# X-rayLaser/DistributedLLM

Measured on NVIDIA H100. Metric: decode tokens/sec LLaMA-7B Q4_0 seq512 bs1, higher is better.
Workload: dtype q4_0*q8_0->f32

## Files before the change

distributedllm_b200/csrc/common.cuh:

```cuda
#pragma once
#include <cuda_runtime.h>
#include <cuda_fp16.h>
#include <cstdint>
#include <cstdio>
#include <cstdarg>
#include <string>

#include "../../include/b200_slice.h"

namespace b200 {

inline std::string & last_error_ref() { static thread_local std::string e; return e; }
inline int fail(int code, const char * fmt, ...) {
    char buf[1024];
    va_list ap; va_start(ap, fmt); vsnprintf(buf, sizeof buf, fmt, ap); va_end(ap);
    last_error_ref() = buf;
    return code;
}
#define B200_CUDA(expr) do { cudaError_t e_ = (expr); if (e_ != cudaSuccess) \
    return b200::fail(B200_ECUDA, "%s failed: %s (%s:%d)", #expr, cudaGetErrorString(e_), __FILE__, __LINE__); } while (0)

__device__ __forceinline__ float fmul(float a, float b) { return __fmul_rn(a, b); }
__device__ __forceinline__ float fadd(float a, float b) { return __fadd_rn(a, b); }
__device__ __forceinline__ float fsub(float a, float b) { return __fsub_rn(a, b); }
__device__ __forceinline__ float ffma(float a, float b, float c) { return __fmaf_rn(a, b, c); }
__device__ __forceinline__ float h2f(uint16_t h) { return __half2float(__ushort_as_half(h)); }
__device__ __forceinline__ uint16_t f2h(float f) { return __half_as_ushort(__float2half_rn(f)); }

__device__ __forceinline__ uint32_t smem_u32(const void * p) { return (uint32_t) __cvta_generic_to_shared(p); }

__device__ __forceinline__ void mbar_init(uint64_t * bar, uint32_t count) {
    asm volatile("mbarrier.init.shared::cta.b64 [%0], %1;" :: "r"(smem_u32(bar)), "r"(count) : "memory");
}
__device__ __forceinline__ void mbar_fence_init() {
    asm volatile("fence.mbarrier_init.release.cluster;" ::: "memory");
}
__device__ __forceinline__ void mbar_arrive(uint64_t * bar) {
    asm volatile("{ .reg .b64 st; mbarrier.arrive.shared::cta.b64 st, [%0]; }" :: "r"(smem_u32(bar)) : "memory");
}
__device__ __forceinline__ void mbar_arrive_expect_tx(uint64_t * bar, uint32_t bytes) {
    asm volatile("{ .reg .b64 st; mbarrier.arrive.expect_tx.shared::cta.b64 st, [%0], %1; }"
                 :: "r"(smem_u32(bar)), "r"(bytes) : "memory");
}
__device__ __forceinline__ bool mbar_try_wait(uint64_t * bar, uint32_t parity) {
    uint32_t ok;
    asm volatile("{ .reg .pred p; mbarrier.try_wait.parity.shared::cta.b64 p, [%1], %2; selp.u32 %0, 1, 0, p; }"
                 : "=r"(ok) : "r"(smem_u32(bar)), "r"(parity) : "memory");
    return ok != 0;
}
__device__ __forceinline__ void mbar_wait(uint64_t * bar, uint32_t parity) {
    while (!mbar_try_wait(bar, parity)) { }
}
__device__ __forceinline__ void bulk_g2s(void * dst_smem, const void * src_gmem, uint32_t bytes, uint64_t * bar) {
    uint64_t pol;
    asm volatile("createpolicy.fractional.L2::evict_first.b64 %0, 1.0;" : "=l"(pol));
    asm volatile("cp.async.bulk.shared::cluster.global.mbarrier::complete_tx::bytes.L2::cache_hint [%0], [%1], %2, [%3], %4;"
                 :: "r"(smem_u32(dst_smem)), "l"(src_gmem), "r"(bytes), "r"(smem_u32(bar)), "l"(pol) : "memory");
}
__device__ __forceinline__ float4 ldg_keep(const float * p) {
    uint64_t pol; float4 v;
    asm volatile("createpolicy.fractional.L2::evict_last.b64 %0, 1.0;" : "=l"(pol));
    asm volatile("ld.global.L2::cache_hint.v4.f32 {%0, %1, %2, %3}, [%4], %5;"
                 : "=f"(v.x), "=f"(v.y), "=f"(v.z), "=f"(v.w) : "l"(p), "l"(pol));
    return v;
}
__device__ __forceinline__ void grid_dep_wait()   { asm volatile("griddepcontrol.wait;" ::: "memory"); }
__device__ __forceinline__ void grid_dep_launch() { asm volatile("griddepcontrol.launch_dependents;" ::: "memory"); }

__device__ __forceinline__ unsigned long long gtime() { unsigned long long t; asm volatile("mov.u64 %0, %%globaltimer;" : "=l"(t)); return t; }
#define B200_TRACE(ptr, slot) do { if (ptr) (ptr)[((size_t) blockIdx.y * gridDim.x + blockIdx.x) * 8 + (slot)] = b200::gtime(); } while (0)

__device__ __forceinline__ void named_bar_sync(int id, int nthreads) {
    asm volatile("bar.sync %0, %1;" :: "r"(id), "r"(nthreads) : "memory");
}

}
```

distributedllm_b200/csrc/kernels.cuh:

```cuda
#pragma once
#include "common.cuh"

namespace b200 {

constexpr int kWT_F16 = 1, kWT_Q4_0 = 2, kWT_Q4_1 = 3, kWT_Q5_0 = 6, kWT_Q5_1 = 7, kWT_Q8_0 = 8;
constexpr int kQ4Chunk = 576, kQ41Chunk = 640, kQ50Chunk = 704, kQ51Chunk = 768, kQ8Chunk = 1088;
constexpr int kWPC = 4;
constexpr int kConsumers = kWPC * 32;
constexpr int kQS = 4;
constexpr float kMagic = 12582912.0f;
constexpr int kMagicI = 0x4B400000;

struct WtTraits {
    int block_bytes;
    int chunk_bytes;
    bool is_signed;
    bool min_plane;
    bool high_plane;
    bool q8_1;
    float act_scale;
};
__host__ __device__ constexpr WtTraits wt_traits(int wt) {
    return wt == kWT_Q4_0 ? WtTraits{18, kQ4Chunk, true, false, false, false, 0.0625f}
         : wt == kWT_Q4_1 ? WtTraits{20, kQ41Chunk, false, true, false, true, 0.0625f}
         : wt == kWT_Q5_0 ? WtTraits{22, kQ50Chunk, true, false, true, false, 0.125f}
         : wt == kWT_Q5_1 ? WtTraits{24, kQ51Chunk, false, true, true, true, 0.125f}
         : wt == kWT_Q8_0 ? WtTraits{34, kQ8Chunk, true, false, false, false, 1.0f}
         :                  WtTraits{0, 0, false, false, false, false, 0.0f};
}
__host__ __device__ constexpr bool wt_block_quant(int wt) { return wt_traits(wt).block_bytes != 0; }
__host__ __device__ constexpr int chunk_bytes(int wt) { return wt_traits(wt).chunk_bytes; }
__host__ __device__ constexpr bool wt_nibbles(int wt) { return wt == kWT_Q4_0 || wt == kWT_Q4_1 || wt == kWT_Q5_0 || wt == kWT_Q5_1; }
__host__ __device__ constexpr bool wt_q8_1(int wt) { return wt_traits(wt).q8_1; }
__host__ __device__ constexpr float wt_act_scale(int wt) { return wt_traits(wt).act_scale; }
__host__ __device__ constexpr int wt_scale_off(int wt) { return wt == kWT_Q8_0 ? 1024 : (wt_traits(wt).high_plane ? 640 : 512); }
__host__ __device__ constexpr int wt_min_off(int wt) { return wt_scale_off(wt) + 64; }
static_assert(chunk_bytes(kWT_Q4_0) == 32 * 18 && chunk_bytes(kWT_Q4_1) == 32 * 20 && chunk_bytes(kWT_Q5_0) == 32 * 22 &&
              chunk_bytes(kWT_Q5_1) == 32 * 24 && chunk_bytes(kWT_Q8_0) == 32 * 34, "a chunk holds the file's bytes, nothing added");
static_assert(kQ50Chunk % 16 == 0 && kQ51Chunk % 16 == 0, "a ring stage stays one bulk copy");

__device__ __forceinline__ uint32_t spread4_hi(uint32_t b) { return (b * 0x10204080u) & 0x80808080u; }

struct PackedW {
    const uint8_t * data;
    int wtype, rows, K, nb, nbq, TR, n_tiles;
    long long tile_bytes;
};

struct RepackArgs {
    const uint8_t * src[3];
    int mode, wtype, rows_per_src, nb, nbq, TR, n_tiles;
    uint8_t * dst;
};

__global__ void k_repack(RepackArgs a) {
    const int cb = chunk_bytes(a.wtype), words = cb / 4;
    const long long total = (long long) a.n_tiles * a.nbq * a.TR * words;
    for (long long i = blockIdx.x * (long long) blockDim.x + threadIdx.x; i < total; i += (long long) gridDim.x * blockDim.x) {
        const int wi = (int)(i % words);
        long long c = i / words;
        const int rg = (int)(c % a.TR); c /= a.TR;
        const int q = (int)(c % a.nbq);
        const int tile = (int)(c / a.nbq);
        const int gi = tile * a.TR + rg;
        int s, sg;
        if (a.mode == 1)      { const int gps = a.rows_per_src / 8; s = gi / gps; sg = gi % gps; }
        else if (a.mode == 2) { s = gi & 1; sg = gi >> 1; }
        else                  { s = 0; sg = gi; }
        const int bsz = wt_traits(a.wtype).block_bytes;
        uint32_t out = 0;
        const bool src_ok = s < 3 && a.src[s] != nullptr;
        if (wt_traits(a.wtype).high_plane) {
            const bool q51 = a.wtype == kWT_Q5_1;
            const int qh_off = q51 ? 4 : 2, qs_off = qh_off + 4;
            if (wi < 128) {
                const int lane = wi >> 2, bq = wi & 3, r = lane >> 2, w = lane & 3;
                const int row = sg * 8 + r, b = q * 4 + bq;
                if (src_ok && row < a.rows_per_src && b < a.nb) {
                    const uint16_t * p = (const uint16_t *)(a.src[s] + ((long long) row * a.nb + b) * bsz + qs_off + 4 * w);
                    out = (uint32_t) p[0] | ((uint32_t) p[1] << 16);
                }
            } else if (wi < 160) {
                const int lane = wi - 128, r = lane >> 2, w = lane & 3, row = sg * 8 + r;
                for (int bq = 0; bq < 4; bq++) {
                    const int b = q * 4 + bq;
                    if (src_ok && row < a.rows_per_src && b < a.nb) {
                        const uint16_t * p = (const uint16_t *)(a.src[s] + ((long long) row * a.nb + b) * bsz + qh_off);
                        const uint32_t qh = (uint32_t) p[0] | ((uint32_t) p[1] << 16);
                        out |= (((qh >> (4 * w)) & 15u) | (((qh >> (16 + 4 * w)) & 15u) << 4)) << (8 * bq);
                    }
                }
            } else {
                const int sel = (wi - 160) >> 4;
                const int h0 = ((wi - 160) & 15) * 2;
                uint32_t v[2] = {0, 0};
                for (int k = 0; k < 2; k++) {
                    const int r = (h0 + k) >> 2, bq = (h0 + k) & 3, row = sg * 8 + r, b = q * 4 + bq;
                    if (src_ok && row < a.rows_per_src && b < a.nb)
                        v[k] = *(const uint16_t *)(a.src[s] + ((long long) row * a.nb + b) * bsz + 2 * sel);
                }
// ... 1013 lines not shown
    for (int i = 0; i < nwarp; i++) S += redd[i];
    const float inv = (float)(1.0 / S);
    for (int t = tid; t < tcount; t += blockDim.x) p16[t] = f2h(fmul(sc[t], inv));
    __syncthreads();

    const int npT = T & ~31;
    const int g = tid / D, c = tid - g * D;
    if (g < 4) {
        float acc[8] = {0.f, 0.f, 0.f, 0.f, 0.f, 0.f, 0.f, 0.f};
        const uint16_t * v = vcb + h * D + c;
        const int lim = min(npT, tcount);
        for (int base = 8 * g; base < lim; base += 32) {
            #pragma unroll
            for (int l = 0; l < 8; l++) {
                const int t = base + l;
                if (t < lim) acc[l] = ffma(h2f(v[(size_t) t * E]), h2f(p16[t]), acc[l]);
            }
        }
        #pragma unroll
        for (int l = 0; l < 8; l++) part[(g * D + c) * 8 + l] = acc[l];
    }
    __syncthreads();
    if (tid < D) {
        float vv[8];
        #pragma unroll
        for (int l = 0; l < 8; l++) {
            const float a0 = fadd(part[(0 * D + tid) * 8 + l], part[(2 * D + tid) * 8 + l]);
            const float a1 = fadd(part[(1 * D + tid) * 8 + l], part[(3 * D + tid) * 8 + l]);
            vv[l] = fadd(a0, a1);
        }
        const float t0 = fadd(vv[0], vv[4]), t1 = fadd(vv[1], vv[5]), t2 = fadd(vv[2], vv[6]), t3 = fadd(vv[3], vv[7]);
        double sumf = (double) fadd(fadd(t0, t1), fadd(t2, t3));
        const uint16_t * v = vcb + h * D + tid;
        for (int t = npT; t < tcount; t++) sumf += (double) fmul(h2f(v[(size_t) t * E]), h2f(p16[t]));
        a.out[(size_t) n * E + h * D + tid] = (float) sumf;
    }
}

struct Attn128Args {
    const float * qkv;
    const uint16_t * q16;
    uint16_t * kc; uint16_t * vc;
    const int * n_past; int E, H, N, n0;
    const float2 * cs; const uint16_t * texp;
    float * out;
    int * aq_out; float * da_out; int out_nbq; float out_dscale;
    int out_soff;
    int n_ctx; float kq_scale;
    unsigned long long * trace;
    const int2 * cols; size_t sess_stride;
    const int * col_T;
    int pf_rows;
    int lut_smem;
};

constexpr int kAttnRow = 272;

__device__ __forceinline__ void cp_async16(void * dst_smem, const void * src) {
    asm volatile("cp.async.cg.shared.global [%0], [%1], 16;" :: "r"(smem_u32(dst_smem)), "l"(src) : "memory");
}
__device__ __forceinline__ void cp_async_wait_all() {
    asm volatile("cp.async.commit_group;" ::: "memory");
    asm volatile("cp.async.wait_group 0;" ::: "memory");
}

__device__ __forceinline__ void cluster_sync_all() {
    asm volatile("barrier.cluster.arrive.release.aligned;" ::: "memory");
    asm volatile("barrier.cluster.wait.acquire.aligned;" ::: "memory");
}
__device__ __forceinline__ void cluster_arrive_relaxed() { asm volatile("barrier.cluster.arrive.relaxed.aligned;" ::: "memory"); }
__device__ __forceinline__ void cluster_wait()           { asm volatile("barrier.cluster.wait.acquire.aligned;" ::: "memory"); }
__device__ __forceinline__ uint32_t dsmem_addr(const void * local, int rank) {
    uint32_t r;
    asm volatile("mapa.shared::cluster.u32 %0, %1, %2;" : "=r"(r) : "r"(smem_u32(local)), "r"(rank));
    return r;
}
__device__ __forceinline__ void dsmem_st(uint32_t addr, float v) {
    asm volatile("st.shared::cluster.f32 [%0], %1;" :: "r"(addr), "f"(v) : "memory");
}
__device__ __forceinline__ void dsmem_st4(uint32_t addr, float4 v) {
    asm volatile("st.shared::cluster.v4.f32 [%0], {%1, %2, %3, %4};" :: "r"(addr), "f"(v.x), "f"(v.y), "f"(v.z), "f"(v.w) : "memory");
}

template <bool FUSE>
__global__ void __cluster_dims__(4, 1, 1) __launch_bounds__(256) k_attn128(const Attn128Args a) {
    extern __shared__ __align__(16) uint8_t smem[];
    __shared__ __align__(16) uint16_t q16s[128], k16s[128], v16s[128];
    __shared__ double redd[8]; __shared__ float redf[8];
    __shared__ __align__(16) float partl[4 * 8 * 32];
    __shared__ __align__(8) uint64_t lutbar;
    if (threadIdx.x == 0) { B200_TRACE(a.trace, 0); grid_dep_launch(); }
    cluster_arrive_relaxed();
    if (!FUSE) grid_dep_wait();
    const int h = blockIdx.x >> 2, g = blockIdx.x & 3, ny = blockIdx.y, n = a.n0 + ny, E = a.E;
    int T, tcount, pos;
    uint16_t * kc = a.kc, * vc = a.vc;
    if (a.cols) {
        const int2 c = a.cols[n]; pos = c.y; tcount = pos + 1; T = (!FUSE && a.col_T) ? a.col_T[n] : tcount;
        kc += (size_t) c.x * a.sess_stride; vc += (size_t) c.x * a.sess_stride;
    }
    else { const int n_past = *a.n_past; T = n_past + a.N; tcount = n_past + n + 1; pos = n_past + n; }
    float * sc = (float *) smem;
    uint16_t * p16 = (uint16_t *)(sc + ((T + 3) & ~3));
    const int tid = threadIdx.x, warp = tid >> 5, lane = tid & 31;
    uint8_t * Ks = smem + ((((size_t)((a.n_ctx + 3) & ~3) * 4 + (size_t)((a.n_ctx + 7) & ~7) * 2) + 15) & ~(size_t) 15);
    uint8_t * Vs = Ks + (size_t) a.pf_rows * kAttnRow;
// ... 144 lines not shown
        for (int tb = 8 * g + l; tb < lim; tb += 128) {
            uint4 vv4[4];
            #pragma unroll
            for (int u = 0; u < 4; u++) {
                const int t = tb + 32 * u;
                const int i = ((t >> 5) << 3) + l;
                const uint16_t * vrow = (FUSE && t == pos) ? v16s : (i < npf ? (const uint16_t *)(Vs + (size_t) i * kAttnRow)
                                                                              : vc + (size_t) t * E + h * 128);
                vv4[u] = t < lim ? *(const uint4 *)(vrow + 8 * cg) : make_uint4(0, 0, 0, 0);
            }
            #pragma unroll
            for (int u = 0; u < 4; u++) {
                const int t = tb + 32 * u;
                if (t < lim) {
                    const uint32_t u4[4] = {vv4[u].x, vv4[u].y, vv4[u].z, vv4[u].w};
                    const float p = h2f(p16[t]);
                    #pragma unroll
                    for (int e = 0; e < 8; e++) {
                        const uint16_t vh = (uint16_t)(u4[e >> 1] >> (16 * (e & 1)));
                        acc[e] = ffma(h2f(vh), p, acc[e]);
                    }
                }
            }
        }
        const uint32_t dst = dsmem_addr(partl + (g * 8 + l) * 32 + 8 * (cg & 3), cg >> 2);
        dsmem_st4(dst, make_float4(acc[0], acc[1], acc[2], acc[3]));
        dsmem_st4(dst + 16, make_float4(acc[4], acc[5], acc[6], acc[7]));
    }
    __syncthreads();
    cluster_sync_all();
    if (threadIdx.x == 0) B200_TRACE(a.trace, 7);

    if (tid < 32) {
        const int c = 32 * g + tid;
        float vv[8];
        #pragma unroll
        for (int l = 0; l < 8; l++) {
            const float p0 = partl[(0 * 8 + l) * 32 + tid], p1 = partl[(1 * 8 + l) * 32 + tid];
            const float p2 = partl[(2 * 8 + l) * 32 + tid], p3 = partl[(3 * 8 + l) * 32 + tid];
            vv[l] = fadd(fadd(p0, p2), fadd(p1, p3));
        }
        const float t0 = fadd(vv[0], vv[4]), t1 = fadd(vv[1], vv[5]), t2 = fadd(vv[2], vv[6]), t3 = fadd(vv[3], vv[7]);
        double sumf = (double) fadd(fadd(t0, t1), fadd(t2, t3));
        for (int t = npT; t < tcount; t++) {
            const uint16_t vh = (FUSE && t == pos) ? v16s[c] : (FUSE ? ((const uint16_t *)(Vt + (size_t)(t - npT) * 64))[tid]
                                                                     : vc[(size_t) t * E + h * 128 + c]);
            sumf += (double) fmul(h2f(vh), h2f(p16[t]));
        }
        const float ov = (float) sumf;
        a.out[(size_t) n * E + h * 128 + c] = ov;
        if (a.aq_out) warp_quant_block(ov, lane, a.aq_out + (size_t) n * a.out_nbq * 32, a.da_out + (size_t) n * a.out_nbq * 4,
                                       4 * h + g, a.out_dscale, a.out_soff);
    }
    if (threadIdx.x == 0) B200_TRACE(a.trace, 3);
}

struct PeerRecvArgs {
    MailboxHdr * mine;
    const uint2 * inbox;
    size_t slot_elems;
    int * peer_ack;
    float * dst; int count;
};

__global__ void __launch_bounds__(1024) k_peer_recv(const PeerRecvArgs a) {
    if (threadIdx.x == 0) grid_dep_launch();
    grid_dep_wait();
    const int s = a.mine->seq_in + 1;
    const uint2 * src = a.inbox + (size_t)(s & (kMbSlots - 1)) * a.slot_elems;
    const unsigned long long t0 = gtime();
    for (int i = blockIdx.x * blockDim.x + threadIdx.x; i < a.count; i += gridDim.x * blockDim.x) {
        uint2 v = ld_ll(src + i);
        while ((int) v.y != s) {
            if (gtime() - t0 > kMbTimeoutNs) { a.mine->err = 1; break; }
            v = ld_ll(src + i);
        }
        a.dst[i] = __uint_as_float(v.x);
    }
    __syncthreads();
    if (threadIdx.x == 0) {
        if (gridDim.x == 1 || atomicAdd(&a.mine->cnt_recv, 1) == (int) gridDim.x - 1) {
            a.mine->cnt_recv = 0;
            a.mine->seq_in = s;
            st_relaxed_sys(a.peer_ack, s);
        }
    }
}

struct PeerSendArgs {
    MailboxHdr * mine;
    uint2 * peer_inbox;
    size_t slot_elems;
    const float * src; int count;
};

__global__ void __launch_bounds__(1024) k_peer_send(const PeerSendArgs a) {
    if (threadIdx.x == 0) grid_dep_launch();
    grid_dep_wait();
    const int s = a.mine->seq_out + 1;
    if (threadIdx.x == 0) mb_wait_slot_free(a.mine, s);
    __syncthreads();
    uint2 * dst = a.peer_inbox + (size_t)(s & (kMbSlots - 1)) * a.slot_elems;
    for (int i = blockIdx.x * blockDim.x + threadIdx.x; i < a.count; i += gridDim.x * blockDim.x) st_ll(dst + i, a.src[i], s);
    __syncthreads();
    if (threadIdx.x == 0) {
        if (gridDim.x == 1 || atomicAdd(&a.mine->cnt_send, 1) == (int) gridDim.x - 1) { a.mine->cnt_send = 0; a.mine->seq_out = s; }
// ... 189 lines not shown
```

distributedllm_b200/csrc/runtime.cu:

```cuda
#include "kernels.cuh"
#include "kquant.cuh"
#include "fastgemm2.cuh"
#include "ggjt_file.hpp"

#include <algorithm>
#include <atomic>
#include <chrono>
#include <climits>
#include <cmath>
#include <condition_variable>
#include <dlfcn.h>
#include <cstdlib>
#include <map>
#include <memory>
#include <mutex>
#include <thread>
#include <type_traits>
#include <vector>

namespace b200 {

constexpr int kSmemLimit = 226 * 1024;

struct LayerW {
    PackedW qkv{}, wo{}, w13{}, w2{};
    PackedW qkv_more[2]{}; int qkv_row[2] = {0, 0};
    uint16_t * f_q = nullptr, * f_k = nullptr, * f_v = nullptr, * f_o = nullptr, * f_1 = nullptr, * f_2 = nullptr, * f_3 = nullptr;
    float * attn_norm = nullptr, * ffn_norm = nullptr;
};

struct GraphKey { const float * in; float * out; int host; bool operator<(const GraphKey & o) const {
    return in != o.in ? in < o.in : (out != o.out ? out < o.out : host < o.host); } };

}

using namespace b200;

struct b200_slice {
    int device = 0, n_sm = 132;
    cudaStream_t stream = nullptr;
    int E = 0, H = 0, D = 0, FF = 0, L = 0, first_layer = 0, n_ctx = 512, wtype = 0;
    int n_sessions = 1, cur = 0;
    std::vector<int> past;
    int * d_npast = nullptr;
    size_t sess_stride = 0;
    struct Seg { int session, past, count, col; };
    std::vector<Seg> segs; std::vector<int> h_pass;
    int * d_pass = nullptr; const int2 * cols = nullptr; const int * col_T = nullptr; const int2 * d_segs = nullptr;
    const AttnTile * d_tiles = nullptr; int n_tiles = 0, tile_rows = 0;
    std::vector<LayerW> layers;
    std::vector<void *> allocs;
    uint16_t * kc = nullptr, * vc = nullptr, * q16 = nullptr;
    float * xa = nullptr, * xb = nullptr, * qkv = nullptr, * att = nullptr, * ffin = nullptr, * gate = nullptr;
    float * d_in = nullptr, * d_out = nullptr, * h_in = nullptr, * h_out = nullptr;
    float2 * cs = nullptr; uint16_t * texp = nullptr, * tsilu = nullptr;
    int * aq_att = nullptr, * aq_gate = nullptr; float * da_att = nullptr, * da_gate = nullptr;
    int nbqE = 0, nbqF = 0;
    int soffE = 0, soffF = 0;
    int * aq_x = nullptr; float * da_x = nullptr; int * nq_counter = nullptr; double * nq_partial = nullptr;
    std::map<GraphKey, cudaGraphExec_t> graphs;
    cudaEvent_t ev0 = nullptr, ev1 = nullptr; bool timed = false;
    int64_t launches = 0, weight_bytes = 0;
    bool use_ring = true, use_graph = true, use_pdl = false, use_nq = true, f16_ring = true, use_tiled_attn = true, f16_mc = true; int f16_mc_cols = 4;
    bool skip_attention = false;
    bool attn_lut_smem = true;
    bool fast_prefill = false; int fast_min_tokens = 32; uint16_t * xh = nullptr;
    int opt_ns = 0, opt_cta_per_sm = 0, opt_nc = 0, opt_pre = 3, opt_nomath = 0;
    float ema_token_ms = 0.f;
    std::mutex mu;
    bool profiling = false; int cur_class = 0;
    std::vector<cudaEvent_t> prof_ev; std::vector<int> prof_cls; size_t prof_used = 0;
    cudaEvent_t mark[2] = {nullptr, nullptr};
    unsigned long long * trace = nullptr; int trace_next = 0; std::vector<int> trace_cls, trace_ctas;
    void * nccl_comm = nullptr; int pp_rank = 0, pp_world = 1; float * d_final = nullptr;
    uint8_t * mb_block = nullptr; size_t mb_slot_floats = 0;
    uint8_t * mb_next = nullptr, * mb_prev = nullptr; bool mb_on = false;
    bool send_pending = false; PeerSendArgs send_args{}; int send_ctas = 1;
    bool fold_send = false, use_fold = true;
    int * kq_aq = nullptr; float * kq_ad = nullptr;
    std::map<GraphKey, cudaGraphExec_t> pp_graphs;
    const b200_stream * owner = nullptr;
};

namespace b200 {

static int env_int(const char * name, int dflt) { const char * v = getenv(name); return v ? atoi(v) : dflt; }

template <typename T> static int dev_alloc(b200_slice * s, T ** p, size_t n) {
    void * q = nullptr;
    cudaError_t e = cudaMalloc(&q, n * sizeof(T));
    if (e != cudaSuccess) return fail(B200_ECUDA, "cudaMalloc(%zu) failed: %s", n * sizeof(T), cudaGetErrorString(e));
    s->allocs.push_back(q); *p = (T *) q; return 0;
}

static void prof_begin(b200_slice * s) {
    if (!s->profiling) return;
    if (s->prof_used + 2 > s->prof_ev.size()) {
        for (int i = 0; i < 2; i++) { cudaEvent_t e; cudaEventCreate(&e); s->prof_ev.push_back(e); }
    }
    cudaEventRecord(s->prof_ev[s->prof_used], s->stream);
}
static void prof_end(b200_slice * s) {
    if (!s->profiling) return;
    cudaEventRecord(s->prof_ev[s->prof_used + 1], s->stream);
    s->prof_cls.push_back(s->cur_class);
    s->prof_used += 2;
}

template <typename K, typename... A>
static int launch(b200_slice * s, K kern, dim3 grid, dim3 block, size_t smem, const A &... args) {
    cudaLaunchConfig_t cfg{};
    cfg.gridDim = grid; cfg.blockDim = block; cfg.dynamicSmemBytes = smem; cfg.stream = s->stream;
    cudaLaunchAttribute at[1];
    at[0].id = cudaLaunchAttributeProgrammaticStreamSerialization;
    at[0].val.programmaticStreamSerializationAllowed = 1;
    cfg.attrs = at; cfg.numAttrs = s->use_pdl ? 1 : 0;
    prof_begin(s);
    B200_CUDA(cudaLaunchKernelEx(&cfg, kern, args...));
// ... 195 lines not shown
        void * p = nullptr;
        cudaDriverEntryPointQueryResult qres;
        if (cudaGetDriverEntryPoint("cuTensorMapEncodeTiled", &p, cudaEnableDefault, &qres) == cudaSuccess && qres == cudaDriverEntryPointSuccess)
            fn = (TensorMapEncodeFn) p;
    });
    return fn;
}

template <int WT, int EPI, int NT>
static int launch_fast_gemm_t(b200_slice * s, const PackedW & W, const float * resid, int ldr, float * y, int ldy, int N, int out_rows) {
    TensorMapEncodeFn enc = tensor_map_encode();
    if (!enc) return fail(B200_ECUDA, "cuTensorMapEncodeTiled is not available from this driver");
    CUtensorMap map;
    const cuuint64_t dims[2] = {(cuuint64_t) W.K, (cuuint64_t) N};
    const cuuint64_t strides[1] = {(cuuint64_t) W.K * 2};
    const cuuint32_t box[2] = {64, (cuuint32_t) NT};
    const cuuint32_t estr[2] = {1, 1};
    CUresult cr = enc(&map, CU_TENSOR_MAP_DATA_TYPE_FLOAT16, 2, (void *) s->xh, dims, strides, box, estr, CU_TENSOR_MAP_INTERLEAVE_NONE,
                      CU_TENSOR_MAP_SWIZZLE_128B, CU_TENSOR_MAP_L2_PROMOTION_L2_256B, CU_TENSOR_MAP_FLOAT_OOB_FILL_NONE);
    if (cr != CUDA_SUCCESS) return fail(B200_ECUDA, "cuTensorMapEncodeTiled failed (%d) for K=%d N=%d", (int) cr, W.K, N);
    if (int rc = smem_attr<k_gemm_tc2<WT, EPI, NT>>(s, f2_smem(WT, NT))) return rc;
    FastGemm2Args a{}; a.W = W; a.resid = resid; a.ldr = ldr; a.y = y; a.ldy = ldy; a.N = N; a.out_rows = out_rows; a.tsilu = s->tsilu;
    const int groups = W.n_tiles * W.TR;
    return launch(s, k_gemm_tc2<WT, EPI, NT>, dim3((groups + 15) / 16, (N + NT - 1) / NT, 1), dim3(kF2Threads, 1, 1), f2_smem(WT, NT), a, map);
}

template <int EPI>
static int launch_fast_gemm(b200_slice * s, const PackedW & W, const float * resid, int ldr, float * y, int ldy, int N, int out_rows) {
    const int mtiles = (W.n_tiles * W.TR + 15) / 16;
    const bool wide = (long long) mtiles * ((N + 255) / 256) >= s->n_sm || N <= 128;
    if (W.wtype == kWT_Q4_0) return wide ? launch_fast_gemm_t<kWT_Q4_0, EPI, 256>(s, W, resid, ldr, y, ldy, N, out_rows)
                                         : launch_fast_gemm_t<kWT_Q4_0, EPI, 128>(s, W, resid, ldr, y, ldy, N, out_rows);
    return wide ? launch_fast_gemm_t<kWT_Q8_0, EPI, 256>(s, W, resid, ldr, y, ldy, N, out_rows)
                : launch_fast_gemm_t<kWT_Q8_0, EPI, 128>(s, W, resid, ldr, y, ldy, N, out_rows);
}

struct AttnSmem { int pf_rows; size_t plain, staged, lut, generic; };

static AttnSmem attn_smem(int n_ctx, int D) {
    AttnSmem m;
    const size_t sc = (size_t)((n_ctx + 3) & ~3) * 4 + (size_t)((n_ctx + 7) & ~7) * 2, sc16 = (sc + 15) & ~(size_t) 15;
    m.pf_rows = std::min(8 * ((n_ctx + 31) / 32), 128);
    m.plain = sc16 + 64;
    m.staged = sc16 + (size_t) 2 * m.pf_rows * kAttnRow + 32 * 64 + 64;
    m.lut = m.staged + 65536;
    m.generic = sc + (size_t) 4 * D * 8 * 4 + 64;
    return m;
}

static bool seg_tiled(const b200_slice * s, const b200_slice::Seg & g) {
    return s->D == 128 && s->use_tiled_attn && g.count > 1 && g.past + g.count <= kAttnTMax;
}

static int attention(b200_slice * s, int il, int N, bool preq) {
    if (s->skip_attention) return 0;
    const int E = s->E, H = s->H, D = s->D;
    const size_t sess_off = s->cols ? 0 : (size_t) s->cur * s->sess_stride;
    uint16_t * kc = s->kc + sess_off + (size_t) il * s->n_ctx * E, * vc = s->vc + sess_off + (size_t) il * s->n_ctx * E;
    int * d_npast = s->d_npast + s->cur;
    const AttnSmem am = attn_smem(s->n_ctx, D);
    const float kq_scale = 1.0f / sqrtf((float) E / (float) H);
    int rc;
    if (D != 128) {
        s->cur_class = 1;
        RopeArgs ra{s->qkv, E, H, D, N, d_npast, s->cs, s->q16, kc, vc, s->cols, s->sess_stride};
        if ((rc = launch(s, k_rope_append, dim3((E / 2 + 255) / 256, N, 1), dim3(256, 1, 1), 0, ra))) return rc;
        s->cur_class = 2;
        AttnArgs aa{s->q16, kc, vc, d_npast, E, H, D, N, s->texp, s->att, kq_scale, s->cols, s->sess_stride, s->col_T};
        return launch(s, k_attention, dim3(H, N, 1), dim3(512, 1, 1), am.generic, aa);
    }
    constexpr int kChunk = 1024;
    Attn128Args aa{};
    aa.pf_rows = am.pf_rows;
    aa.qkv = s->qkv; aa.q16 = s->q16; aa.kc = kc; aa.vc = vc; aa.n_past = d_npast; aa.E = E; aa.H = H; aa.N = N;
    aa.cols = s->cols; aa.sess_stride = s->sess_stride;
    aa.cs = s->cs; aa.texp = s->texp; aa.out = s->att;
    aa.n_ctx = s->n_ctx; aa.kq_scale = kq_scale;
    const float dsc = preq ? wt_act_scale(s->wtype) : 0.f;
    if (preq) { aa.aq_out = s->aq_att; aa.da_out = s->da_att; aa.out_nbq = s->nbqE; aa.out_dscale = dsc; aa.out_soff = s->soffE; }
    auto launch_tiled = [&](int t_rows, int n_blocks, const AttnTile * tiles) {
        AttnTiledArgs ta{};
        ta.q16 = s->q16; ta.kc = kc; ta.vc = vc; ta.n_past = d_npast; ta.E = E; ta.H = H; ta.N = N; ta.texp = s->texp; ta.out = s->att;
        if (preq) { ta.aq_out = s->aq_att; ta.da_out = s->da_att; ta.out_nbq = s->nbqE; ta.out_dscale = dsc; ta.out_soff = s->soffE; }
        ta.kq_scale = kq_scale; ta.t_rows = t_rows; ta.t_pad = (t_rows + 31) & ~31;
        ta.tiles = tiles; ta.sess_stride = s->sess_stride;
        const size_t tsm = (size_t) ta.t_rows * kAttnRow + (size_t) kAttnQB * ta.t_pad * 6 + 4 * 8 * 128 * 4 + kAttnQB * 256 + 64;
        if (int e = smem_attr<k_attn128_tiled>(s, kSmemLimit)) return e;
        return launch(s, k_attn128_tiled, dim3(H, n_blocks, 1), dim3(512, 1, 1), tsm, ta);
    };
    auto launch_fused_cols = [&](int c0, int cnt) {
        for (int n0 = 0; n0 < cnt; n0 += kChunk) {
            aa.n0 = c0 + n0;
            if (int e = launch(s, k_attn128<true>, dim3(4 * H, std::min(cnt - n0, kChunk), 1), dim3(256, 1, 1), am.staged, aa)) return e;
        }
        return 0;
    };
    if (s->cols && !s->col_T) {
        s->cur_class = 2;
        return launch_fused_cols(0, N);
    }
    if (s->cols) {
        const std::vector<b200_slice::Seg> & sg = s->segs;
        s->cur_class = 2;
        for (size_t k = 0; k < sg.size();) {
            size_t e = k;
            while (e < sg.size() && sg[e].count == 1) e++;
            if (e > k && (rc = launch_fused_cols(sg[k].col, sg[e - 1].col + 1 - sg[k].col))) return rc;
            k = e + 1;
        }
        s->cur_class = 1;
        for (const b200_slice::Seg & g : sg) {
            if (g.count == 1) continue;
            RopeArgs ra{s->qkv + (size_t) g.col * 3 * E, E, H, D, g.count, d_npast, s->cs, s->q16 + (size_t) g.col * E, kc, vc,
                        s->cols + g.col, s->sess_stride};
            if ((rc = launch(s, k_rope_append, dim3((E / 2 + 255) / 256, g.count, 1), dim3(256, 1, 1), 0, ra))) return rc;
        }
        s->cur_class = 2;
        if (s->n_tiles && (rc = launch_tiled(s->tile_rows, s->n_tiles, s->d_tiles))) return rc;
        aa.col_T = s->col_T;
        for (const b200_slice::Seg & g : sg) {
            if (g.count == 1 || seg_tiled(s, g)) continue;
            for (int n0 = 0; n0 < g.count; n0 += kChunk) {
                aa.n0 = g.col + n0;
                if ((rc = launch(s, k_attn128<false>, dim3(4 * H, std::min(g.count - n0, kChunk), 1), dim3(256, 1, 1), am.plain, aa))) return rc;
            }
        }
        return 0;
    }
    if (N == 1) {
        s->cur_class = 2;
        aa.n0 = 0;
        if (s->trace && s->trace_next < 512) { aa.trace = s->trace + (size_t) s->trace_next * 1024 * 8; s->trace_next++; s->trace_cls.push_back(2); s->trace_ctas.push_back(4 * H); }
        aa.lut_smem = s->attn_lut_smem;
        return launch(s, k_attn128<true>, dim3(4 * H, 1, 1), dim3(256, 1, 1), aa.lut_smem ? am.lut : am.staged, aa);
    }
    s->cur_class = 1;
    RopeArgs ra{s->qkv, E, H, D, N, d_npast, s->cs, s->q16, kc, vc, nullptr, 0};
    if ((rc = launch(s, k_rope_append, dim3((E / 2 + 255) / 256, N, 1), dim3(256, 1, 1), 0, ra))) return rc;
    s->cur_class = 2;
    if (s->use_tiled_attn && s->past[s->cur] + N <= kAttnTMax)
        return launch_tiled(s->past[s->cur] + N, (N + kAttnQB - 1) / kAttnQB, nullptr);
    for (int n0 = 0; n0 < N; n0 += kChunk) {
        aa.n0 = n0;
        const int cnt = N - n0 < kChunk ? N - n0 : kChunk;
        if ((rc = launch(s, k_attn128<false>, dim3(4 * H, cnt, 1), dim3(256, 1, 1), am.plain, aa))) return rc;
    }
    return 0;
}


static int layer_f16(b200_slice * s, int il, int N, const float * cur, float * nxt) {
    const int E = s->E, FF = s->FF;
    const LayerW & Lw = s->layers[il];
    int rc;
    GemvF16Args q{}; q.K = E; q.x = cur; q.ldx = E; q.norm_w = Lw.attn_norm; q.N = N; q.tsilu = s->tsilu;
    q.rows = 3 * E; q.ldy = 3 * E;
    q.W = Lw.f_q; q.y = s->qkv;
    if ((rc = launch_f16<PRO_NORM, EPI_STORE>(s, q))) return rc;
    if ((rc = attention(s, il, N, false))) return rc;
    s->cur_class = 3;
    GemvF16Args o{}; o.K = E; o.x = s->att; o.ldx = E; o.N = N; o.tsilu = s->tsilu;
    o.rows = E; o.W = Lw.f_o; o.resid = cur; o.ldr = E; o.y = s->ffin; o.ldy = E;
    if ((rc = launch_f16<PRO_PLAIN, EPI_RESID>(s, o))) return rc;
    s->cur_class = 4;
    GemvF16Args g{}; g.K = E; g.x = s->ffin; g.ldx = E; g.norm_w = Lw.ffn_norm; g.N = N; g.tsilu = s->tsilu;
    g.rows = FF; g.W = Lw.f_1; g.W2 = Lw.f_3; g.y = s->gate; g.ldy = FF;
    if ((rc = launch_f16<PRO_NORM, EPI_GATE>(s, g))) return rc;
    s->cur_class = 5;
    GemvF16Args w{}; w.K = FF; w.x = s->gate; w.ldx = FF; w.N = N; w.tsilu = s->tsilu;
    w.rows = E; w.W = Lw.f_2; w.resid = s->ffin; w.ldr = E; w.y = nxt; w.ldy = E;
    return launch_f16<PRO_PLAIN, EPI_RESID>(s, w);
}

static int layer_exact(b200_slice * s, int il, int N, const float * cur, float * nxt) {
    const int E = s->E, FF = s->FF;
    const LayerW & Lw = s->layers[il];
    const bool nq = s->use_nq && N == 1 && !s->cols && Lw.wo.n_tiles <= 256 && Lw.wo.n_tiles <= s->n_sm * 2;
    const float dsc = wt_act_scale(s->wtype);
    int rc;
    GemvArgs q{}; q.W = Lw.qkv; q.x = cur; q.ldx = E; q.norm_w = Lw.attn_norm; q.y = s->qkv; q.ldy = 3 * E;
    q.N = N; q.out_rows = 3 * E; q.tsilu = s->tsilu; q.aq_in = s->aq_x; q.da_in = s->da_x; q.in_soff = s->soffE;
    if (N > 1 && (rc = launch_norm_quant(s, cur, E, Lw.attn_norm, N))) return rc;
    if ((rc = N > 1 || (il > 0 && nq) ? launch_gemv<1, PRO_PREQ, EPI_STORE>(s, q) : launch_gemv<1, PRO_NORM, EPI_STORE>(s, q))) return rc;
    if ((rc = attention(s, il, N, true))) return rc;
    s->cur_class = 3;
    GemvArgs o{}; o.W = Lw.wo; o.x = s->att; o.ldx = E; o.resid = cur; o.ldr = E; o.y = s->ffin; o.ldy = E;
    o.N = N; o.out_rows = E; o.tsilu = s->tsilu; o.aq_in = s->aq_att; o.da_in = s->da_att; o.in_soff = s->soffE; o.out_soff = s->soffE;
    o.nq_norm_w = Lw.ffn_norm; o.nq_counter = s->nq_counter; o.nq_partial = s->nq_partial; o.aq_out = s->aq_x; o.da_out = s->da_x; o.out_nbq = s->nbqE; o.out_dscale = dsc;
    if (s->D == 128) rc = nq ? launch_gemv<1, PRO_PREQ, EPI_RESID_NQ>(s, o) : launch_gemv<1, PRO_PREQ, EPI_RESID>(s, o);
    else             rc = nq ? launch_gemv<1, PRO_PLAIN, EPI_RESID_NQ>(s, o) : launch_gemv<1, PRO_PLAIN, EPI_RESID>(s, o);
    if (rc) return rc;
    s->cur_class = 4;
    GemvArgs g{}; g.W = Lw.w13; g.x = s->ffin; g.ldx = E; g.norm_w = Lw.ffn_norm; g.y = s->gate; g.ldy = FF;
    g.N = N; g.out_rows = FF; g.tsilu = s->tsilu; g.aq_in = s->aq_x; g.da_in = s->da_x; g.in_soff = s->soffE; g.out_soff = s->soffF;
    g.aq_out = s->aq_gate; g.da_out = s->da_gate; g.out_nbq = s->nbqF; g.out_dscale = dsc;
    if (N > 1 && (rc = launch_norm_quant(s, s->ffin, E, Lw.ffn_norm, N))) return rc;
    if ((rc = N > 1 || nq ? launch_gemv<2, PRO_PREQ, EPI_GATEQ>(s, g) : launch_gemv<2, PRO_NORM, EPI_GATEQ>(s, g))) return rc;
    s->cur_class = 5;
    GemvArgs w{}; w.W = Lw.w2; w.resid = s->ffin; w.ldr = E; w.y = nxt; w.ldy = E;
    w.N = N; w.out_rows = E; w.tsilu = s->tsilu; w.aq_in = s->aq_gate; w.da_in = s->da_gate; w.in_soff = s->soffF; w.out_soff = s->soffE;
    if (il + 1 < s->L && nq) {
        w.nq_norm_w = s->layers[il + 1].attn_norm; w.nq_counter = s->nq_counter; w.nq_partial = s->nq_partial; w.aq_out = s->aq_x; w.da_out = s->da_x;
        w.out_nbq = s->nbqE; w.out_dscale = dsc;
        return launch_gemv<1, PRO_PREQ, EPI_RESID_NQ>(s, w);
    }
    if (s->fold_send && il == s->L - 1) return launch_w2_send<false>(s, w);
    return launch_gemv<1, PRO_PREQ, EPI_RESID>(s, w);
}

static int layer_fast(b200_slice * s, int il, int N, const float * cur, float * nxt) {
    const int E = s->E, FF = s->FF;
    const LayerW & Lw = s->layers[il];
    int rc;
    if ((rc = launch_prep<true>(s, cur, E, Lw.attn_norm, E, N))) return rc;
    if ((rc = launch_fast_gemm<FG_STORE>(s, Lw.qkv, nullptr, 0, s->qkv, 3 * E, N, 3 * E))) return rc;
    if ((rc = attention(s, il, N, true))) return rc;
    s->cur_class = 3;
    if ((rc = launch_prep<false>(s, s->att, E, nullptr, E, N))) return rc;
    if ((rc = launch_fast_gemm<FG_RESID>(s, Lw.wo, cur, E, s->ffin, E, N, E))) return rc;
    s->cur_class = 4;
    if ((rc = launch_prep<true>(s, s->ffin, E, Lw.ffn_norm, E, N))) return rc;
    if ((rc = launch_fast_gemm<FG_GATE>(s, Lw.w13, nullptr, 0, s->gate, FF, N, FF))) return rc;
    s->cur_class = 5;
    if ((rc = launch_prep<false>(s, s->gate, FF, nullptr, FF, N))) return rc;
    return launch_fast_gemm<FG_RESID>(s, Lw.w2, s->ffin, E, nxt, E, N, E);
}

static int layer_kquant(b200_slice * s, int il, int N, const float * cur, float * nxt) {
    const int E = s->E, FF = s->FF;
    const LayerW & Lw = s->layers[il];
    int rc;
    GemvArgs q{}; q.W = Lw.qkv; q.x = cur; q.ldx = E; q.norm_w = Lw.attn_norm; q.y = s->qkv; q.ldy = 3 * E;
    q.N = N; q.out_rows = Lw.qkv.rows; q.tsilu = s->tsilu;
    if ((rc = quant_kq(s, q, true)) || (rc = launch_gemv_kq<1, PRO_PREQ, EPI_STORE>(s, q))) return rc;
    for (int i = 0; i < 2 && Lw.qkv_more[i].data; i++) {
        q.W = Lw.qkv_more[i]; q.y = s->qkv + Lw.qkv_row[i]; q.out_rows = Lw.qkv_more[i].rows;
        if ((rc = launch_gemv_kq<1, PRO_PREQ, EPI_STORE>(s, q))) return rc;
// ... 465 lines not shown
    s->sess_stride = (size_t) s->L * nE;
    s->past.assign(s->n_sessions, 0);
    if ((rc = dev_alloc(s, &s->kc, s->n_sessions * s->sess_stride)) || (rc = dev_alloc(s, &s->vc, s->n_sessions * s->sess_stride)) ||
        (rc = dev_alloc(s, &s->d_pass, pass_table_ints(s->n_ctx, s->n_sessions))) ||
        (rc = dev_alloc(s, &s->q16, nE)) || (rc = dev_alloc(s, &s->xa, nE)) || (rc = dev_alloc(s, &s->xb, nE)) ||
        (rc = dev_alloc(s, &s->qkv, 3 * nE)) || (rc = dev_alloc(s, &s->att, nE)) || (rc = dev_alloc(s, &s->ffin, nE)) ||
        (rc = dev_alloc(s, &s->gate, (size_t) s->n_ctx * FF)) || (rc = dev_alloc(s, &s->d_in, nE)) ||
        (rc = dev_alloc(s, &s->d_out, nE)) || (rc = dev_alloc(s, &s->d_npast, (size_t) s->n_sessions)))
        return rc;
    if ((rc = dev_alloc(s, &s->xh, (size_t) s->n_ctx * (FF > E ? FF : E) + 64))) return rc;
    if (wt_kquant(s->wtype)) {
        const int nbq = std::max(s->layers[0].wo.nbq, s->layers[0].w2.nbq);
        if ((rc = dev_alloc(s, &s->kq_aq, (size_t) s->n_ctx * nbq * 72)) || (rc = dev_alloc(s, &s->kq_ad, (size_t) s->n_ctx * kq_nbd(nbq))))
            return rc;
    }
    if (s->wtype != kWT_F16 && !wt_kquant(s->wtype)) {
        s->nbqE = s->layers[0].wo.nbq; s->nbqF = s->layers[0].w2.nbq;
        const size_t nq = (size_t) s->n_ctx;
        const size_t pl = wt_q8_1(s->wtype) ? 2 : 1;
        if (pl == 2) { s->soffE = (int)(nq * s->nbqE * 4); s->soffF = (int)(nq * s->nbqF * 4); }
        if ((rc = dev_alloc(s, &s->aq_att, nq * s->nbqE * 32)) || (rc = dev_alloc(s, &s->da_att, pl * nq * s->nbqE * 4)) ||
            (rc = dev_alloc(s, &s->aq_gate, nq * s->nbqF * 32)) || (rc = dev_alloc(s, &s->da_gate, pl * nq * s->nbqF * 4))) return rc;
        if ((rc = dev_alloc(s, &s->aq_x, nq * s->nbqE * 32)) || (rc = dev_alloc(s, &s->da_x, pl * nq * s->nbqE * 4)) ||
            (rc = dev_alloc(s, &s->nq_counter, 2 * nq)) || (rc = dev_alloc(s, &s->nq_partial, nq * 256))) return rc;
        B200_CUDA(cudaMemset(s->aq_x, 0, nq * s->nbqE * 128)); B200_CUDA(cudaMemset(s->da_x, 0, pl * nq * s->nbqE * 16));
        B200_CUDA(cudaMemset(s->nq_counter, 0, 2 * nq * 4));
        B200_CUDA(cudaMemset(s->aq_att, 0, nq * s->nbqE * 128));  B200_CUDA(cudaMemset(s->da_att, 0, pl * nq * s->nbqE * 16));
        B200_CUDA(cudaMemset(s->aq_gate, 0, nq * s->nbqF * 128)); B200_CUDA(cudaMemset(s->da_gate, 0, pl * nq * s->nbqF * 16));
    }
    B200_CUDA(cudaMemset(s->kc, 0, s->n_sessions * s->sess_stride * 2));
    B200_CUDA(cudaMemset(s->vc, 0, s->n_sessions * s->sess_stride * 2));
    B200_CUDA(cudaMemset(s->d_npast, 0, 4 * (size_t) s->n_sessions));
    B200_CUDA(cudaMallocHost((void **) &s->h_in, (size_t) E * 4));
    B200_CUDA(cudaMallocHost((void **) &s->h_out, (size_t) E * 4));
    lap("KV cache + activations");
    if ((rc = build_tables(s))) return rc;
    lap("exp / SiLU / RoPE tables");
    if (env_int("B200_TRACE", 0)) {
        if ((rc = dev_alloc(s, &s->trace, (size_t) 512 * 1024 * 8))) return rc;
        B200_CUDA(cudaMemset(s->trace, 0, (size_t) 512 * 1024 * 8 * 8));
    }
    B200_CUDA(cudaFuncSetAttribute(k_attention, cudaFuncAttributeMaxDynamicSharedMemorySize, kSmemLimit));
    B200_CUDA(cudaFuncSetAttribute(k_attn128<true>, cudaFuncAttributeMaxDynamicSharedMemorySize, 200 * 1024));
    B200_CUDA(cudaFuncSetAttribute(k_attn128<false>, cudaFuncAttributeMaxDynamicSharedMemorySize, 200 * 1024));
    if (s->D == 128) {
        cudaLaunchConfig_t cfg{};
        cfg.gridDim = dim3(4 * s->H, 1, 1); cfg.blockDim = dim3(256, 1, 1); cfg.dynamicSmemBytes = attn_need;
        int clusters = 0;
        B200_CUDA(cudaOccupancyMaxActiveClusters(&clusters, k_attn128<true>, &cfg));
        s->attn_lut_smem = clusters >= s->H;
        if (ltrace) fprintf(stderr, "[b200 load] single-token attention: %d of %d clusters resident with the exp table in shared memory: %s\n",
                            clusters, s->H, s->attn_lut_smem ? "staged" : "read through L2");
    }
    B200_CUDA(cudaEventCreate(&s->ev0));
    B200_CUDA(cudaEventCreate(&s->ev1));
    B200_CUDA(cudaDeviceSynchronize());
    lap("attributes + final sync");
    if (ltrace) fprintf(stderr, "[b200 load] total %.3f s for %.2f GB of weights\n", tnow() - t_begin, s->weight_bytes / 1e9);
    return 0;
}

static void destroy(b200_slice * s) {
    cudaSetDevice(s->device);
    if (s->stream) cudaStreamSynchronize(s->stream);
    for (auto & kv : s->graphs) cudaGraphExecDestroy(kv.second);
    for (auto & kv : s->pp_graphs) cudaGraphExecDestroy(kv.second);
    if (s->mb_next) cudaIpcCloseMemHandle(s->mb_next);
    if (s->mb_prev && s->mb_prev != s->mb_next) cudaIpcCloseMemHandle(s->mb_prev);
    for (void * p : s->allocs) cudaFree(p);
    if (s->h_in) cudaFreeHost(s->h_in);
    if (s->h_out) cudaFreeHost(s->h_out);
    if (s->ev0) cudaEventDestroy(s->ev0);
    if (s->ev1) cudaEventDestroy(s->ev1);
    for (cudaEvent_t e : s->prof_ev) cudaEventDestroy(e);
    for (int i = 0; i < 2; i++) if (s->mark[i]) cudaEventDestroy(s->mark[i]);
    if (s->stream) cudaStreamDestroy(s->stream);
    delete s;
}

static int refuse_owned(const b200_slice * s) {
    return fail(B200_EINVAL, "the handle belongs to the open generation stream %p: b200_stream_close it first", (const void *) s->owner);
}
#define B200_UNOWNED(h) do { if ((h)->owner) return b200::refuse_owned(h); } while (0)

}

extern "C" {

const char * b200_last_error(void) { return b200::last_error_ref().c_str(); }
const char * b200_version(void) { return "b200-slice 0.1 (sm_90a, exact mode)"; }

int b200_slice_load(const char * path, int device, int n_ctx, b200_slice_t ** out) {
    return b200_slice_load_ex(path, device, n_ctx, 1, out);
}

int b200_slice_load_ex(const char * path, int device, int n_ctx, int n_sessions, b200_slice_t ** out) {
    if (!path || !out) return fail(B200_EINVAL, "b200_slice_load: null argument");
    *out = nullptr;
    if (n_sessions < 1 || n_sessions > 4096) return fail(B200_EINVAL, "n_sessions %d outside [1, 4096]", n_sessions);
    int ndev = 0;
    if (cudaGetDeviceCount(&ndev) != cudaSuccess || ndev == 0)
        return fail(B200_ENODEV, "no CUDA device visible: the slice forward has no CPU fallback");
    if (device < 0 || device >= ndev) return fail(B200_ENODEV, "device %d out of range (%d visible)", device, ndev);
    cudaDeviceProp prop;
    B200_CUDA(cudaGetDeviceProperties(&prop, device));
    if (prop.major != 9 || prop.minor != 0) return fail(B200_ENODEV, "device %d is sm_%d%d; this library is built for sm_90a only", device, prop.major, prop.minor);
// ... 1843 lines not shown
```

Baseline: 554.2.

## Prefetch leading bytes of each FFN w13 tile into L2 from attention kernel

```diff
diff --git a/distributedllm_b200/csrc/common.cuh b/distributedllm_b200/csrc/common.cuh
--- a/distributedllm_b200/csrc/common.cuh
+++ b/distributedllm_b200/csrc/common.cuh
@@ -57,6 +57,9 @@
     asm volatile("cp.async.bulk.shared::cluster.global.mbarrier::complete_tx::bytes.L2::cache_hint [%0], [%1], %2, [%3], %4;"
                  :: "r"(smem_u32(dst_smem)), "l"(src_gmem), "r"(bytes), "r"(smem_u32(bar)), "l"(pol) : "memory");
 }
+__device__ __forceinline__ void bulk_prefetch_l2(const void * src, uint32_t bytes) {
+    asm volatile("cp.async.bulk.prefetch.L2.global [%0], %1;" :: "l"(src), "r"(bytes) : "memory");
+}
 __device__ __forceinline__ float4 ldg_keep(const float * p) {
     uint64_t pol; float4 v;
     asm volatile("createpolicy.fractional.L2::evict_last.b64 %0, 1.0;" : "=l"(pol));
diff --git a/distributedllm_b200/csrc/kernels.cuh b/distributedllm_b200/csrc/kernels.cuh
--- a/distributedllm_b200/csrc/kernels.cuh
+++ b/distributedllm_b200/csrc/kernels.cuh
@@ -46,6 +46,14 @@
     int wtype, rows, K, nb, nbq, TR, n_tiles;
     long long tile_bytes;
 };
+
+struct L2Lead {
+    const uint8_t * data; long long tile_bytes; int n_tiles; uint32_t lead;
+};
+__device__ __forceinline__ void l2_lead_prefetch(const L2Lead & p, int cta, int ncta) {
+    if (p.lead == 0) return;
+    for (int t = cta; t < p.n_tiles; t += ncta) bulk_prefetch_l2(p.data + (long long) t * p.tile_bytes, p.lead);
+}
 
 struct RepackArgs {
     const uint8_t * src[3];
@@ -1165,6 +1173,7 @@
     const int * col_T;
     int pf_rows;
     int lut_smem;
+    L2Lead pf_w13;
 };
 
 constexpr int kAttnRow = 272;
@@ -1415,6 +1424,7 @@
         if (a.aq_out) warp_quant_block(ov, lane, a.aq_out + (size_t) n * a.out_nbq * 32, a.da_out + (size_t) n * a.out_nbq * 4,
                                        4 * h + g, a.out_dscale, a.out_soff);
     }
+    if (FUSE && tid == 255) l2_lead_prefetch(a.pf_w13, blockIdx.y * gridDim.x + blockIdx.x, gridDim.x * gridDim.y);
     if (threadIdx.x == 0) B200_TRACE(a.trace, 3);
 }
 
diff --git a/distributedllm_b200/csrc/runtime.cu b/distributedllm_b200/csrc/runtime.cu
--- a/distributedllm_b200/csrc/runtime.cu
+++ b/distributedllm_b200/csrc/runtime.cu
@@ -64,6 +64,7 @@
     bool use_ring = true, use_graph = true, use_pdl = false, use_nq = true, f16_ring = true, use_tiled_attn = true, f16_mc = true; int f16_mc_cols = 4;
     bool skip_attention = false;
     bool attn_lut_smem = true;
+    uint32_t lead_w13 = 0;
     bool fast_prefill = false; int fast_min_tokens = 32; uint16_t * xh = nullptr;
     int opt_ns = 0, opt_cta_per_sm = 0, opt_nc = 0, opt_pre = 3, opt_nomath = 0;
     float ema_token_ms = 0.f;
@@ -365,7 +366,7 @@
     return s->D == 128 && s->use_tiled_attn && g.count > 1 && g.past + g.count <= kAttnTMax;
 }
 
-static int attention(b200_slice * s, int il, int N, bool preq) {
+static int attention(b200_slice * s, int il, int N, bool preq, const L2Lead & pf_w13 = L2Lead{}) {
     if (s->skip_attention) return 0;
     const int E = s->E, H = s->H, D = s->D;
     const size_t sess_off = s->cols ? 0 : (size_t) s->cur * s->sess_stride;
@@ -445,6 +446,7 @@
         aa.n0 = 0;
         if (s->trace && s->trace_next < 512) { aa.trace = s->trace + (size_t) s->trace_next * 1024 * 8; s->trace_next++; s->trace_cls.push_back(2); s->trace_ctas.push_back(4 * H); }
         aa.lut_smem = s->attn_lut_smem;
+        aa.pf_w13 = pf_w13;
         return launch(s, k_attn128<true>, dim3(4 * H, 1, 1), dim3(256, 1, 1), aa.lut_smem ? am.lut : am.staged, aa);
     }
     s->cur_class = 1;
@@ -458,6 +460,18 @@
         const int cnt = N - n0 < kChunk ? N - n0 : kChunk;
         if ((rc = launch(s, k_attn128<false>, dim3(4 * H, cnt, 1), dim3(256, 1, 1), am.plain, aa))) return rc;
     }
+    return 0;
+}
+
+constexpr long long kW13LeadBytes = 10ll << 20;
+
+static int size_w13_lead(b200_slice * s) {
+    if (s->wtype != kWT_Q4_0 || s->layers.empty()) return 0;
+    int l2 = 0;
+    B200_CUDA(cudaDeviceGetAttribute(&l2, cudaDevAttrL2CacheSize, s->device));
+    const PackedW & W = s->layers[0].w13;
+    const long long stage = (long long) kQS * W.TR * chunk_bytes(W.wtype), budget = std::min(kW13LeadBytes, (long long) l2 / 2);
+    if (W.n_tiles > 0) s->lead_w13 = (uint32_t) std::min(budget / W.n_tiles / stage * stage, W.tile_bytes);
     return 0;
 }
 
@@ -495,7 +509,8 @@
     q.N = N; q.out_rows = 3 * E; q.tsilu = s->tsilu; q.aq_in = s->aq_x; q.da_in = s->da_x; q.in_soff = s->soffE;
     if (N > 1 && (rc = launch_norm_quant(s, cur, E, Lw.attn_norm, N))) return rc;
     if ((rc = N > 1 || (il > 0 && nq) ? launch_gemv<1, PRO_PREQ, EPI_STORE>(s, q) : launch_gemv<1, PRO_NORM, EPI_STORE>(s, q))) return rc;
-    if ((rc = attention(s, il, N, true))) return rc;
+    const bool warm = N == 1 && !s->cols;
+    if ((rc = attention(s, il, N, true, L2Lead{Lw.w13.data, Lw.w13.tile_bytes, Lw.w13.n_tiles, warm ? s->lead_w13 : 0u}))) return rc;
     s->cur_class = 3;
     GemvArgs o{}; o.W = Lw.wo; o.x = s->att; o.ldx = E; o.resid = cur; o.ldr = E; o.y = s->ffin; o.ldy = E;
     o.N = N; o.out_rows = E; o.tsilu = s->tsilu; o.aq_in = s->aq_att; o.da_in = s->da_att; o.in_soff = s->soffE; o.out_soff = s->soffE;
@@ -1067,6 +1082,7 @@
         if (ltrace) fprintf(stderr, "[b200 load] single-token attention: %d of %d clusters resident with the exp table in shared memory: %s\n",
                             clusters, s->H, s->attn_lut_smem ? "staged" : "read through L2");
     }
+    if ((rc = size_w13_lead(s))) return rc;
     B200_CUDA(cudaEventCreate(&s->ev0));
     B200_CUDA(cudaEventCreate(&s->ev1));
     B200_CUDA(cudaDeviceSynchronize());
```

After: 555.0 (median of 6 runs). No clear change (+0.1%).
